# AIDynamicAction/rcognita

Hardware: AMD Instinct MI355X
Metric: env-control-steps/sec (whole node), 3wrobot Nactor=10 (higher is better)
Workload: dtype f64

## Files before the change

include/rcg.h:

```cpp
#ifndef RCG_H
#define RCG_H

#include <stdint.h>

#ifdef __cplusplus
extern "C" {
#endif

#define RCG_VERSION 124

#define RCG_MAX_DS 5
#define RCG_MAX_DU 2
#define RCG_MAX_CHI 7
#define RCG_MAX_PARS 5
#define RCG_MAX_DC 35
#define RCG_MAX_ROW 64
#define RCG_MAX_NACTOR 4096

typedef enum rcg_status {
  RCG_OK = 0,
  RCG_ERR_BAD_ARG = -1,
  RCG_ERR_HIP = -2,
  RCG_ERR_NO_DEVICE = -3,
  RCG_ERR_UNSUPPORTED = -4,
// ... 178 lines not shown
  RCG_KID_ACTOR = 1,
  RCG_KID_ACTOR_DMA = 2,
  RCG_KID_TICKS = 3,
  RCG_KID_ACTOR_OPT = 4,
  RCG_KID_NOMINAL = 5,
  RCG_KID_SIM = 6,
  RCG_KID_SIM_V = 7,
  RCG_KID_SIM_DIST = 8,
  RCG_KID_CRITIC_FIT = 9,
  RCG_KID_ACTOR_DMA_PACKED = 10,
  RCG_KID_ACTOR_SEARCH = 11,
  RCG_KID_COUNT_ = 12
} rcg_kernel_id;
int rcg_last_launch(const rcg_handle* h, int32_t kind, int32_t* kernel_id, int32_t* variant, int32_t* envs_per_wave);
int rcg_last_launch_zero_w(const rcg_handle* h, int32_t kind, uint32_t* mask);
const char* rcg_kernel_name(int32_t kernel_id);

#ifdef __cplusplus
}
#endif
#endif
```

rcognita_amd/_native.py:

```python
from __future__ import annotations

import ctypes as C
import os
import sys

_HERE = os.path.dirname(os.path.abspath(__file__))
LIB_PATH = os.path.join(_HERE, "lib", "librcg.so")

RCG_VERSION = 124
OK, ERR_BAD_ARG, ERR_HIP, ERR_NO_DEVICE, ERR_UNSUPPORTED, ERR_NONFINITE = 0, -1, -2, -3, -4, -5
SYS_3WROBOT, SYS_3WROBOT_NI, SYS_2TANK = 0, 1, 2
MODE_MPC, MODE_RQL, MODE_SQL = 0, 1, 2
STAGE_QUADRATIC, STAGE_BIQUADRATIC = 0, 1
CRITIC_QUAD_LIN, CRITIC_QUADRATIC, CRITIC_QUAD_NOMIX, CRITIC_QUAD_MIX = 0, 1, 2, 3
F32, F64 = 0, 1
HOST, DEVICE = 0, 1
FLAG_HAS_TARGET, FLAG_PER_ENV_PARS, FLAG_REF_LAG, FLAG_ACCUM_EVERY_SUBSTEP, FLAG_NO_CLIP = 1, 2, 4, 8, 16
FLAG_DISTURB = 32
DIM_DISTURB = {0: 2, 1: 2, 2: 1}

(FIELD_STATE, FIELD_ACTION, FIELD_ACCUM, FIELD_STEP_IDX, FIELD_EPISODE_IDX, FIELD_STATUS, FIELD_PARS,
 FIELD_STATE_INIT, FIELD_STATE_PREV, FIELD_BEST_J, FIELD_BEST_IDX, FIELD_W_CRITIC, FIELD_W_PREV, FIELD_OBS_BUF,
 FIELD_ACT_BUF, FIELD_RETURNS, FIELD_ACTION_SQN, FIELD_DISTURB, FIELD_SUBSTEP_IDX) = range(19)
FIELD_COUNT = 19
# ... 6 lines not shown
SYS_DIMS = {SYS_3WROBOT: (5, 2, 2), SYS_3WROBOT_NI: (3, 2, 0), SYS_2TANK: (2, 1, 5)}
SYS_DY = {}
SYS_USER_BASE = 16
MAX_DS, MAX_DU, MAX_PARS = 5, 2, 5

SYMBOLS = [
    "rcg_version", "rcg_last_error", "rcg_device_count", "rcg_create", "rcg_destroy", "rcg_set_stream", "rcg_use_own_stream",
    "rcg_synchronize", "rcg_dev_alloc", "rcg_dev_free", "rcg_memcpy_h2d", "rcg_memcpy_d2h", "rcg_set_field",
    "rcg_get_field", "rcg_field_bytes", "rcg_field_ptr", "rcg_rhs", "rcg_stage_obj", "rcg_critic",
    "rcg_actor_cost", "rcg_critic_cost", "rcg_sim_step", "rcg_sim_step_h", "rcg_actor_argmin", "rcg_control_tick",
    "rcg_critic_update", "rcg_control_ticks", "rcg_control_tick_n", "rcg_actor_optimize", "rcg_control_tick_opt", "rcg_nominal_action",
    "rcg_control_tick_nominal", "rcg_rhs_full", "rcg_disturb_noise", "rcg_episode_reset", "rcg_episode_stats", "rcg_tick_count", "rcg_set_tick_count", "rcg_profile", "rcg_profile_read",
    "rcg_profile_samples", "rcg_last_launch", "rcg_kernel_name", "rcg_wait_stream", "rcg_nominal_theta", "rcg_set_optimizer", "rcg_set_optimizer_tol", "rcg_set_tick_parts", "rcg_join", "rcg_loop_step", "rcg_loop_step_begin", "rcg_loop_step_end",
    "rcg_actor_search", "rcg_control_tick_search", "rcg_candidates_sample", "rcg_release_stream",
    "rcg_register_system", "rcg_rtc_version", "rcg_system_info", "rcg_system_output_info", "rcg_out",
    "rcg_system_has_critic", "rcg_system_programs", "rcg_critic_fit", "rcg_last_launch_zero_w", "rcg_system_has_search",
]
KERNEL_ACTOR, KERNEL_SIM, KERNEL_CRITIC = 0, 1, 2
(KID_NONE, KID_ACTOR, KID_ACTOR_DMA, KID_TICKS, KID_ACTOR_OPT, KID_NOMINAL, KID_SIM, KID_SIM_V, KID_SIM_DIST,
 KID_CRITIC_FIT, KID_ACTOR_DMA_PACKED, KID_ACTOR_SEARCH) = range(12)
DMA_MPC_G1, DMA_MPC, DMA_RQL_0, DMA_SQL_0 = 0, 1, 2, 6
LOOP_DECIDE, LOOP_PUSH, LOOP_FIT = 1, 2, 4
DMA_RQL_GEN_0 = 12
DMA_MPC_GEND, DMA_MPC_GENF = 10, 11


class RcgCfg(C.Structure):

    _fields_ = [
        ("struct_size", C.c_int32), ("sys_id", C.c_int32), ("batch", C.c_int32), ("dtype", C.c_int32),
        ("device", C.c_int32), ("n_actor", C.c_int32), ("mode", C.c_int32), ("stage_obj_struct", C.c_int32),
# ... 86 lines not shown
        "rcg_candidates_sample": (C.c_int, [vp, vp, i32, i32, vp]),
        "rcg_nominal_action": (C.c_int, [vp, vp, vp, vp, i32, C.c_double, C.POINTER(C.c_double), i32]),
        "rcg_control_tick_nominal": (C.c_int, [vp, C.c_double, C.POINTER(C.c_double)]),
        "rcg_nominal_theta": (C.c_int, [vp, vp, vp, i32]),
        "rcg_rhs_full": (C.c_int, [vp, vp, vp, vp, vp, vp, vp, vp, i32, i32]),
        "rcg_disturb_noise": (C.c_int, [vp, vp, vp]),
        "rcg_episode_reset": (C.c_int, [vp]),
        "rcg_episode_stats": (C.c_int, [vp, i32, vp, C.POINTER(RcgSummary)]),
        "rcg_tick_count": (i64, [vp]),
        "rcg_set_tick_count": (C.c_int, [vp, i64]),
        "rcg_profile": (C.c_int, [vp, i32]),
        "rcg_profile_read": (C.c_int, [vp, i32, C.POINTER(C.c_double), C.POINTER(i64)]),
        "rcg_profile_samples": (C.c_int, [vp, i32, C.POINTER(C.c_double), i64, C.POINTER(i64)]),
        "rcg_last_launch": (C.c_int, [vp, i32, C.POINTER(i32), C.POINTER(i32), C.POINTER(i32)]),
        "rcg_last_launch_zero_w": (C.c_int, [vp, i32, C.POINTER(C.c_uint32)]),
        "rcg_kernel_name": (C.c_char_p, [i32]),
        "rcg_wait_stream": (C.c_int, [vp, vp]),
        "rcg_release_stream": (C.c_int, [vp, vp]),
        "rcg_register_system": (C.c_int, [C.c_char_p, C.c_char_p, i32, i32, i32, C.POINTER(i32)]),
        "rcg_rtc_version": (C.c_int, [C.POINTER(i32), C.POINTER(i32)]),
        "rcg_system_info": (C.c_int, [i32, C.POINTER(i32), C.POINTER(i32), C.POINTER(i32), C.POINTER(i32)]),
        "rcg_system_output_info": (C.c_int, [i32, C.POINTER(i32), C.POINTER(i32), C.POINTER(i32)]),
        "rcg_out": (C.c_int, [vp, vp, vp, i32]),
        "rcg_system_has_critic": (C.c_int, [i32, C.POINTER(i32)]),
        "rcg_system_has_search": (C.c_int, [i32, C.POINTER(i32)]),
        "rcg_critic_fit": (C.c_int, [vp]),
        "rcg_system_programs": (C.c_int, [i32, C.c_char_p, i64, C.POINTER(i64)]),
    }
    for name, (res, args) in sig.items():
        fn = getattr(L, name)
# ... 55 lines not shown
```

rcognita_amd/csrc/rcg_actor_dma.hpp:

```cpp
#pragma once
#include <hip/hip_ext.h>
#include "rcg_kernels.hpp"

#ifndef RCG_DMA_AUX
#define RCG_DMA_AUX 2
#endif
#ifndef RCG_DMA_PRIO
#define RCG_DMA_PRIO 0
#endif

namespace rcg {

enum : int {
  DMA_MPC_G1 = 0,
  DMA_MPC = 1,
  DMA_RQL_0 = 2 ,
  DMA_SQL_0 = 6 ,
  DMA_MPC_GEND = 10,
  DMA_MPC_GENF = 11,
  DMA_RQL_GEN_0 = 12 ,
  DMA_VARIANTS = 16
};
__host__ __device__ constexpr bool dma_is_sql(int v) { return v >= DMA_SQL_0 && v < DMA_MPC_GEND; }
__host__ __device__ constexpr bool dma_is_rql(int v) { return (v >= DMA_RQL_0 && v < DMA_SQL_0) || v >= DMA_RQL_GEN_0; }
// ... 34 lines not shown
#else
  const double Jmin = wave_min_f64(bestJ);
  bestI = (int)wave_min_u32(bestJ == Jmin ? (unsigned)bestI : 0x7fffffffu);
  bestJ = Jmin;
#endif
}

template <typename Sys, typename real>
__host__ __device__ constexpr unsigned dma_zw_preset() {
  if constexpr (sizeof(real) == 8 && !HasOut<Sys>::value)
    return Sys::ZW_PRESET;
  else
    return 0u;
}

template <typename S, typename = void>
struct HasPrefix {
  static constexpr bool value = false;
};
template <typename S>
struct HasPrefix<S, void_t_<decltype(S::PFX_FREE)>> {
  static constexpr bool value = true;
};
template <typename S>
constexpr unsigned pfx_free() {
  if constexpr (HasPrefix<S>::value)
    return S::PFX_FREE;
  else
    return 0u;
}
template <typename S>
constexpr int pfx_heading() {
  if constexpr (HasPrefix<S>::value)
    return S::PFX_HEADING;
  else
    return -1;
}

__device__ __forceinline__ float uniform_r(float v) {
  return __uint_as_float((unsigned)__builtin_amdgcn_readfirstlane((int)__float_as_uint(v)));
}
__device__ __forceinline__ double uniform_r(double v) {
  const unsigned long long b = (unsigned long long)__double_as_longlong(v);
  const unsigned lo = (unsigned)__builtin_amdgcn_readfirstlane((int)(unsigned)b);
  const unsigned hi = (unsigned)__builtin_amdgcn_readfirstlane((int)(unsigned)(b >> 32));
  return __longlong_as_double((long long)(((unsigned long long)hi << 32) | lo));
}

template <int J, int NP, int SZ, int PIECE>
__device__ __forceinline__ void dma_pieces(const unsigned char* g, unsigned off, unsigned char* l) {
  typedef __attribute__((address_space(3))) void lds_void;
  typedef const __attribute__((address_space(1))) void glb_void;
  if constexpr (J < NP) {
    constexpr int BASE = (J * PIECE / 4096) * 4096;
    const unsigned char* const gb = g + (off + (unsigned)BASE);
    if constexpr (SZ == 16)
      __builtin_amdgcn_global_load_lds((glb_void*)gb, (lds_void*)(l + BASE), 16, J * PIECE - BASE, RCG_DMA_AUX);
    else
      __builtin_amdgcn_global_load_lds((glb_void*)gb, (lds_void*)(l + BASE), 4, J * PIECE - BASE, RCG_DMA_AUX);
    dma_pieces<J + 1, NP, SZ, PIECE>(g, off, l);
  }
}

__host__ __device__ constexpr int dma_rpl(int r, int esz) { return r * esz <= 24 ? 4 : (r * esz <= 32 ? 2 : 1); }

template <typename Sys, typename real, int R, bool TGT, int V, unsigned ZW = 0u>
__global__ __launch_bounds__(256) void k_actor_dma(const ActorArgs<real> A, const KParams<real> P) {
  constexpr int DS = Sys::DS, DY = sys_dy<Sys>(), DU = Sys::DU, NCHI = DY + DU, NP = Sys::NP;
  constexpr bool OUT = HasOut<Sys>::value;
  constexpr bool G1 = V == DMA_MPC_G1, SQL = dma_is_sql(V), RQL = dma_is_rql(V), CRIT = RQL || SQL;
  constexpr bool GEND = V == DMA_MPC_GEND, GENF = V == DMA_MPC_GENF, GEN = GEND || GENF;
  constexpr bool GENR = V >= DMA_RQL_GEN_0;
  static_assert(!(GEN || GENR) || TGT, "the generic-cost instances subtract a target (zeros for a handle without one)");
  static_assert(ZW == 0u || (G1 && sizeof(real) == 8 && !OUT && ZW == Sys::ZW_PRESET),
                "the zero-weight instance: DMA_MPC_G1, float64, no output map, the policy's preset mask");
  constexpr int CS = dma_cs(V);
  constexpr int DCMAX = CRIT ? dma_dc(CS, DY, DU) : 1;
  constexpr int ESZ = (int)sizeof(real);
  constexpr int WSLOT = dma_wslot(ESZ, V, DY, DU);
  constexpr bool WLDS = WSLOT > 0;
  constexpr int WREG = WLDS ? 1 : DCMAX;
  static_assert(R % DU == 0 && R >= DU && R <= 40, "row = N*du reals, at most 40 (f32: 160 bytes, f64: 320)");
  constexpr int N = R / DU;
  constexpr bool PFX = HasPrefix<Sys>::value && !OUT;
  constexpr unsigned FREE = PFX ? pfx_free<Sys>() : 0u;
  constexpr int HD = PFX ? pfx_heading<Sys>() : -1;
  constexpr bool TRIG0 = PFX && HD >= 0 && N >= 2;
  constexpr bool TRIG1 = TRIG0 && ((FREE >> (HD >= 0 ? HD : 0)) & 1u) && N >= 3;
  constexpr int RPL = dma_rpl(R, ESZ), TROWS = 64 * RPL;
  constexpr int TILE = TROWS * R * ESZ;
// ... 51 lines not shown
          __builtin_amdgcn_global_load_lds((glb_void*)(g + (o4 + (unsigned)(NFULL * 1024 + j * 256))),
                                           (lds_void*)(tile + NFULL * 1024 + j * 256), 4, 0, RCG_DMA_AUX);
    }
  };
  const int last_rows = rem_rows ? rem_rows : TROWS;
  auto rows_of = [&](int tt) -> int { return tt == T - 1 ? last_rows : TROWS; };

  real y0[DY], yn[sys_dxy<Sys>()], x0[DS], xn[DS], pv[NP > 0 ? NP : 1], pn[NP > 0 ? NP : 1], wc[WREG], wn[WREG];
  real wnl = 0;
  const bool lag = A.state_sys != A.obs;
#pragma unroll
  for (int i = 0; i < NP; ++i) pn[i] = P.pars[i];
#pragma unroll
  for (int i = 0; i < WREG; ++i) wn[i] = wc[i] = 0;
  constexpr int dc_rt = CRIT ? DCMAX : 0;
  auto fetch_env = [&](long b) {
    if (RCG_DBG(A, 4)) {
#pragma unroll
      for (int c = 0; c < sys_dxy<Sys>(); ++c) yn[c] = (real)0.5;
#pragma unroll
      for (int c = 0; c < DS; ++c) xn[c] = (real)0.5;
      return;
    }
    if constexpr (OUT) {
      load_obs_raw<Sys, real>(A.obs, A.obs_x, B, b, yn);
    } else {
#pragma unroll
      for (int c = 0; c < DS; ++c) yn[c] = A.obs[(long)c * B + b];
    }
    if (lag) {
#pragma unroll
// ... 66 lines not shown
#pragma unroll
  for (int c = 0; c < DS; ++c) x1s[c] = 0;
#pragma unroll
  for (int c = 0; c < DY; ++c) Sini[c] = 0;
  real bestJ = inf_r<real>();
  int bestI = 0x7fffffff;
  real bu[DU];
#pragma unroll
  for (int c = 0; c < DU; ++c) bu[c] = 0;
  real resJ = 0, resAcc = 0, resU[DU];
  int resI = 0;
#pragma unroll
  for (int c = 0; c < DU; ++c) resU[c] = 0;

  auto adopt_regs = [&]() {
    if constexpr (OUT) {
#pragma unroll
      for (int c = 0; c < DS; ++c) x0[c] = lag ? xn[c] : yn[c];
#pragma unroll
      for (int i = 0; i < NP; ++i) pv[i] = pn[i];
      pre_env = Sys::template prepare<real>(pv);
      obs_of_raw<Sys, real>(pre_env, A.obs_x, yn, y0);
    } else {
#pragma unroll
      for (int c = 0; c < DS; ++c) {
        y0[c] = yn[c];
        x0[c] = lag ? xn[c] : yn[c];
      }
    }
    if (CRIT && WLDS) {
      if (lane < dc_rt) wl[lane] = wnl;
      asm volatile("s_waitcnt lgkmcnt(0)" ::: "memory");
      __builtin_amdgcn_wave_barrier();
    } else if (CRIT) {
#pragma unroll
      for (int i = 0; i < WREG; ++i) wc[i] = wn[i];
    }
  };
  auto adopt_rest = [&]() {
    if constexpr (PFX) {
#pragma unroll
      for (int c = 0; c < DS; ++c) x0[c] = uniform_r(x0[c]);
      if constexpr (TRIG0) {
        sincos_sel<real, true>(x0[HD], &trig0[0], &trig0[1]);
        if constexpr (FREE != 0) {
          real uz[DU], d[DS];
#pragma unroll
          for (int c = 0; c < DU; ++c) uz[c] = 0;
          Sys::template rhs_trig<real>(pre_env, x0, uz, trig0[0], trig0[1], d);
#pragma unroll
          for (int c = 0; c < DS; ++c)
            if ((FREE >> c) & 1u) x1s[c] = uniform_r(fma_r(h, d[c], x0[c]));
        }
        if constexpr (TRIG1) {
          sincos_sel<real, true>(x1s[HD], &trig1[0], &trig1[1]);
          trig1[0] = uniform_r(trig1[0]);
          trig1[1] = uniform_r(trig1[1]);
        }
        if constexpr (FREE == 0) {
          trig0[0] = uniform_r(trig0[0]);
          trig0[1] = uniform_r(trig0[1]);
        }
      }
      if constexpr (G1) {
#pragma unroll
        for (int c = 0; c < DY; ++c) {
          if ((ZW >> c) & 1u) continue;
          const real chi0 = TGT ? y0[c] - P.target[c] : y0[c];
          real a = fma_r(chi0, chi0, (real)0);
          if (N >= 2 && ((FREE >> c) & 1u)) {
            const real chi1 = TGT ? x1s[c] - P.target[c] : x1s[c];
            a = fma_r(chi1, chi1, a);
          }
          Sini[c] = uniform_r(a);
        }
      }
    }
    if constexpr (ZW != 0u) {
      real z = 0;
#pragma unroll
      for (int i = 0; i < DY; ++i)
        if ((ZW >> i) & 1u) z = fma_r(P.R1d[i], y0[i] * y0[i], z);
      zw0 = uniform_r(z);
    }
    bestJ = inf_r<real>();
    bestI = 0x7fffffff;
  };
  const bool adopt_early = OUT || T == 1;

  for (int g = 0; g < n_tiles; ++g) {
    if (t == 0) {
      if constexpr (!OUT) {
        if (env_pars) pre_env = Sys::template prepare<real>(pn);
      }
      if (adopt_early) adopt_regs();
    }
    if constexpr (RCG_DMA_PRIO > 0 && ESZ == 8) __builtin_amdgcn_s_setprio(RCG_DMA_PRIO);
    asm volatile("s_waitcnt vmcnt(0)" ::: "memory");
    real rows[RPL][R];
#pragma unroll
    for (int j = 0; j < RPL; ++j) {
      const real* const myrow = reinterpret_cast<const real*>(tile) + (j * 64 + lane) * R;
#pragma unroll
      for (int i = 0; i < R; ++i) rows[j][i] = myrow[i];
    }
    asm volatile("s_waitcnt lgkmcnt(0)" ::: "memory");
    __builtin_amdgcn_wave_barrier();
// ... 207 lines not shown
```

rcognita_amd/csrc/rcg_api.hip:

```cpp
#include <cstdarg>
#include <cstdio>
#include <cstdlib>
#include <cstring>

#include "rcg_disturb.hpp"
#include "rcg_handle.hpp"
#include "rcg_search.hpp"

using namespace rcg;

static thread_local std::string g_err = "";

int rcg_fail(rcg_handle* h, int code, const char* fmt, ...) {
  char buf[512];
  va_list ap;
  va_start(ap, fmt);
  vsnprintf(buf, sizeof buf, fmt, ap);
  va_end(ap);
  if (h)
    h->err = buf;
  else
    g_err = buf;
  return code;
}
// ... 224 lines not shown
  h->dc = dim_critic(cfg->critic_struct, h->dy, du);
  h->esz = cfg->dtype == RCG_F64 ? 8 : 4;
  h->stream = nullptr;
  h->own_stream = nullptr;
  h->bounce = nullptr;
  h->tick_parts = 0;
  h->split_stream[0] = h->split_stream[1] = nullptr;
  h->split_fork = h->split_join[0] = h->split_join[1] = nullptr;
  h->split_pending = false;
  h->sub_lo = h->sub_hi = 0;
  h->probe = 0;
  h->d_summary = nullptr;
  h->d_const = nullptr;
  h->fit_scratch = nullptr;
  h->fit_scratch_bytes = 0;
  h->loop_seq = 0;
  h->loop_io.on = false;
  h->loop_pending = false;
  h->loop_pin = nullptr;
  h->sqn_alt = nullptr;
  h->loop_pending_decided = false;
  h->prof_mask = 0;
  h->prof_stride = 1;
  memset(h->prof_seen, 0, sizeof h->prof_seen);
  h->tick_count = 0;
  h->opt_ftol = 0.0;
  h->opt_memory = -1;
  h->cur_a = h->cur_b = nullptr;
  h->scope_due = false;
  h->order_ev = nullptr;
// ... 113 lines not shown
  if (h->own_stream) (void)hipStreamDestroy(h->own_stream);
  for (int p = 0; p < 2; ++p) {
    if (h->split_stream[p]) {
      (void)hipStreamSynchronize(h->split_stream[p]);
      (void)hipStreamDestroy(h->split_stream[p]);
    }
    if (h->split_join[p]) (void)hipEventDestroy(h->split_join[p]);
  }
  if (h->split_fork) (void)hipEventDestroy(h->split_fork);
  if (h->bounce) (void)hipHostFree(h->bounce);
  if (h->loop_pin) (void)hipHostFree(h->loop_pin);
  if (h->sqn_alt) (void)hipFree(h->sqn_alt);
  if (h->d_summary) (void)hipFree(h->d_summary);
  if (h->d_const) (void)hipFree(h->d_const);
  if (h->fit_scratch) (void)hipFree(h->fit_scratch);
  for (auto& p : h->ev_pending) {
    (void)hipEventDestroy(p.a);
    (void)hipEventDestroy(p.b);
  }
  for (auto e : h->ev_free) (void)hipEventDestroy(e);
  if (h->order_ev) (void)hipEventDestroy(h->order_ev);
  if (h->release_ev) (void)hipEventDestroy(h->release_ev);
  delete h;
  return RCG_OK;
}

int rcg_set_stream(rcg_handle* h, void* hip_stream) {
  DeviceGuard dev_guard(h);
  if (!h) return RCG_ERR_BAD_ARG;
  if ((hipStream_t)hip_stream == h->stream) return RCG_OK;
// ... 836 lines not shown

int rcg_last_launch(const rcg_handle* h, int32_t kind, int32_t* kernel_id, int32_t* variant, int32_t* envs_per_wave) {
  if (!h || kind < 0 || kind >= RCG_KERNEL_COUNT_) return RCG_ERR_BAD_ARG;
  if (kernel_id) *kernel_id = h->last[kind].kernel_id;
  if (variant) *variant = h->last[kind].variant;
  if (envs_per_wave) *envs_per_wave = h->last[kind].envs_per_wave;
  return RCG_OK;
}

int rcg_last_launch_zero_w(const rcg_handle* h, int32_t kind, uint32_t* mask) {
  if (!h || !mask || kind < 0 || kind >= RCG_KERNEL_COUNT_) return RCG_ERR_BAD_ARG;
  *mask = h->last[kind].zero_w;
  return RCG_OK;
}

const char* rcg_kernel_name(int32_t kernel_id) {
  static const char* const names[RCG_KID_COUNT_] = {"none",        "k_actor",   "k_actor_dma", "k_ticks",    "k_actor_opt",
                                                    "k_nominal",   "k_sim",     "k_sim_v",     "k_sim_dist", "k_critic_fit",
                                                    "k_actor_dma_packed", "k_actor_search"};
  return (kernel_id >= 0 && kernel_id < RCG_KID_COUNT_) ? names[kernel_id] : "?";
}

}
```

rcognita_amd/csrc/rcg_dma_launch.hpp:

```cpp
#pragma once

#include "rcg_actor_dma.hpp"
#include "rcg_actor_dma_packed.hpp"

namespace rcg {

template <typename Sys, typename real, int GROUP, int R>
static bool launch_dma_r(int r, int variant, dim3 grid, dim3 block, size_t lds, hipStream_t s, const ActorArgs<real>& A,
                         const KParams<real>& P, hipEvent_t ev_a, hipEvent_t ev_b) {
  if constexpr (R > dma_max_row<real>()) {
    return false;
  } else {
    if (r != R) return launch_dma_r<Sys, real, GROUP, R + 1>(r, variant, grid, block, lds, s, A, P, ev_a, ev_b);
    if constexpr (R % Sys::DU != 0) {
      return false;
    } else {
#define RCG_DMA_LAUNCH(FN)                                                                                           \
  {                                                                                                                  \
    auto fn = FN;                                                                                                    \
    if (lds > 64 * 1024)      \
      (void)hipFuncSetAttribute(reinterpret_cast<const void*>(fn), hipFuncAttributeMaxDynamicSharedMemorySize,       \
                                (int)lds);                                                                           \
    if (ev_a)                                                                                                        \
      hipExtLaunchKernelGGL(fn, grid, block, (std::uint32_t)lds, s, ev_a, ev_b, 0, A, P);                            \
    else                                                                                                             \
      hipLaunchKernelGGL(fn, grid, block, lds, s, A, P);                                                             \
    return true;                                                                                                     \
  }
#define RCG_DMA_CASE(V) \
  case V:               \
    RCG_DMA_LAUNCH((k_actor_dma<Sys, real, R, ((V) >= DMA_MPC_GEND ? true : Sys::TGT), V>))
      if constexpr (GROUP == 0) {
        constexpr unsigned ZWP = dma_zw_preset<Sys, real>();
        if constexpr (ZWP != 0u) {
          if (dma_zero_w<real>(ZWP, variant, A, P) != 0u) RCG_DMA_LAUNCH((k_actor_dma<Sys, real, R, Sys::TGT, DMA_MPC_G1, ZWP>))
        }
        switch (variant) {
          RCG_DMA_CASE(DMA_MPC_G1)
          RCG_DMA_CASE(DMA_MPC)
        }
      } else if constexpr (GROUP == 6) {
        switch (variant) {
          RCG_DMA_CASE(DMA_MPC_GEND)
          RCG_DMA_CASE(DMA_MPC_GENF)
        }
      } else if constexpr (GROUP == 7) {
        switch (variant) {
          RCG_DMA_CASE(DMA_RQL_GEN_0 + RCG_CRITIC_QUAD_LIN)
          RCG_DMA_CASE(DMA_RQL_GEN_0 + RCG_CRITIC_QUADRATIC)
          RCG_DMA_CASE(DMA_RQL_GEN_0 + RCG_CRITIC_QUAD_NOMIX)
// ... 92 lines not shown
```

rcognita_amd/csrc/rcg_handle.hpp:

```cpp
#pragma once
#include <hip/hip_ext.h>
#include <hip/hip_runtime.h>

#include <cstdint>
#include <cstdio>
#include <cstdlib>
#include <map>
#include <string>
#include <vector>

#include "rcg_actor_opt.hpp"
#include "rcg_kernels.hpp"

struct rcg_handle {
  rcg_cfg cfg;
  int ds, du, np, dc, nchi;
  int dy;
  bool rtc_has_out;
  size_t esz;
  hipStream_t stream;
  hipStream_t own_stream;
  void* f[RCG_FIELD_COUNT_];
  size_t fbytes[RCG_FIELD_COUNT_];
  double* d_summary;
// ... 3 lines not shown
  void* d_const;
  struct {
    bool on;
    const double* act_in;
    int n_substeps, dc;
    double *out, *flag, seq;
  } loop_io;
  bool loop_pending;
  int loop_pending_row;
  bool loop_pending_decided;
  void* sqn_alt;
  void* loop_pin;
  uint64_t loop_seq;
  void* fit_scratch;
  size_t fit_scratch_bytes;
  rcg::KParams<float> p32;
  rcg::KParams<double> p64;
  const struct SysVTable* sys;
  const struct RtcSystem* rtc;
  std::map<std::string, hipFunction_t> rtc_fn;
  std::string err;
  unsigned prof_mask;
  unsigned prof_stride;
  uint64_t prof_seen[RCG_KERNEL_COUNT_];
  std::vector<hipEvent_t> ev_free;
  struct Pending {
    hipEvent_t a, b;
    int kernel;
  };
  std::vector<Pending> ev_pending;
// ... 2 lines not shown
  std::vector<float> prof_samples[RCG_KERNEL_COUNT_];
  hipEvent_t cur_a, cur_b;
  bool scope_due;
  hipEvent_t order_ev;
  hipEvent_t release_ev;
  void* bounce;
  int tick_parts;
  hipStream_t split_stream[2];
  hipEvent_t split_fork, split_join[2];
  bool split_pending;
  int sub_lo, sub_hi;
  int probe;
  struct LastLaunch {
    int32_t kernel_id, variant, envs_per_wave;
    uint32_t zero_w;
  } last[RCG_KERNEL_COUNT_];
};
static constexpr size_t kProfMaxSamples = 65536;

static constexpr size_t kBounceBytes = 16384;
static constexpr int kSplitMinBatch = 65536;
static constexpr int kVariantSplitBit = 4096;
static inline void note_launch(rcg_handle* h, int kind, int kernel_id, int variant, int envs_per_wave) {
  h->last[kind].kernel_id = kernel_id;
  h->last[kind].variant = variant | (h->sub_hi > 0 ? kVariantSplitBit : 0);
  h->last[kind].envs_per_wave = envs_per_wave;
  h->last[kind].zero_w = 0u;
}

static constexpr size_t kConstR64 = 512, kConstW = 1296, kConstBytes = 2256;
static constexpr int kFitMaxRows = 8;

int rcg_fail(rcg_handle* h, int code, const char* fmt, ...);

#define HIPCHK(h, call)                                                                                 \
  do {                                                                                                  \
    hipError_t e_ = (call);                                                                             \
    if (e_ != hipSuccess)                                                                               \
      return rcg_fail((h), RCG_ERR_HIP, "%s failed: %s (%s:%d)", #call, hipGetErrorString(e_), __FILE__, \
                      __LINE__);                                                                        \
  } while (0)

// ... 142 lines not shown
```

rcognita_amd/csrc/rcg_kernels.hpp:

```cpp
#pragma once
#include <stdint.h>

#include <type_traits>

#include "../../include/rcg.h"
#include "rcg_systems.hpp"

namespace rcg {

enum : int { STAGE_FULL = 1, STAGE_BIQUAD = 2 };

#ifdef RCG_DEV
#define RCG_DBG(A, bit) ((A).dbg & (bit))
#else
#define RCG_DBG(A, bit) 0
#endif

template <typename real>
struct KParams {
  real pars[RCG_MAX_PARS];
  real lo[RCG_MAX_DU], hi[RCG_MAX_DU];
  const real* __restrict__ Rfull;
  real R1d[RCG_MAX_CHI], R2d[RCG_MAX_CHI];
  real target[RCG_MAX_DS];
// ... 272 lines not shown
  int G;
  int n_tiles;
  int grid_g;
  int vec_ok;
  int gpw;
  int jwave;
  int no_multi;
  int dbg;
  int env_lo, env_hi;
  real* sim_state;
  real* sim_state_prev;
  const real* sim_action;
  uint32_t* sim_status;
  int sim_n_sub;
  int obs_x;
};

typedef float v4f __attribute__((ext_vector_type(4)));

template <typename real>
__device__ __forceinline__ void stage_tile(const real* __restrict__ g, real* __restrict__ l, int n,
                                           int lane, int vec_ok) {
  if (vec_ok) {
    const int nv = (int)(((long)n * (long)sizeof(real)) >> 4);
    const v4f* __restrict__ gv = reinterpret_cast<const v4f*>(g);
    v4f* __restrict__ lv = reinterpret_cast<v4f*>(l);
    const int nfull = nv >> 6;
    for (int base = 0; base < nfull; base += 8) {
      const int cnt = nfull - base;
      v4f r[8];
// ... 693 lines not shown
  for (int c = 0; c < DU; ++c) u[c] = A.action[(long)c * B + b];
  const auto pre = load_pre<Sys, real>(P, A.pars_env, b);
  real accum = P.accum_every_substep ? A.accum[b] : (real)0;
  if (!env_substeps<Sys, real, TGT>(P, pre, A.n_sub, x, xp, u, st, accum)) {
    A.status[b] = st;
    return;
  }
#pragma unroll
  for (int c = 0; c < DS; ++c) {
    A.state[(long)c * B + b] = x[c];
    A.state_prev[(long)c * B + b] = xp[c];
  }
  if (P.accum_every_substep) A.accum[b] = accum;
}

template <typename Sys, typename real, bool TGT>
__global__ __launch_bounds__(256) void k_sim_v(const SimArgs<real> A, const KParams<real> P) {
  constexpr int DS = Sys::DS, DU = Sys::DU, NP = Sys::NP, VEC = 16 / (int)sizeof(real);
  typedef real vreal __attribute__((ext_vector_type(VEC)));
  typedef uint32_t vu32 __attribute__((ext_vector_type(VEC)));
  const long B = P.B;
  const long b0 = ((long)blockIdx.x * blockDim.x + threadIdx.x) * VEC;
  if (b0 >= B) return;
  vreal xv[DS], uv[DU], pv[NP > 0 ? NP : 1], av;
#pragma unroll
  for (int c = 0; c < DS; ++c) xv[c] = *reinterpret_cast<const vreal*>(A.state + (long)c * B + b0);
#pragma unroll
  for (int c = 0; c < DU; ++c) uv[c] = *reinterpret_cast<const vreal*>(A.action + (long)c * B + b0);
  const vu32 stv = *reinterpret_cast<const vu32*>(A.status + b0);
  if (A.pars_env) {
// ... 229 lines not shown
```

rcognita_amd/csrc/rcg_sysops.hpp:

```cpp
#pragma once
#include <cmath>
#include <cstdlib>
#include <cstring>
#include <type_traits>

#include "rcg_actor_dma.hpp"
#include "rcg_actor_dma_packed.hpp"
#include "rcg_critic_fit_ml.hpp"
#include "rcg_actor_opt.hpp"
#include "rcg_critic_fit.hpp"
#include "rcg_critic_fit_gen.hpp"
#include "rcg_disturb.hpp"
#include "rcg_handle.hpp"
#include "rcg_loop.hpp"
#include "rcg_nominal.hpp"
#include "rcg_search.hpp"
#include "rcg_ticks.hpp"

namespace rcg {

template <typename F>
static int by_dtype(rcg_handle* h, F&& f) {
  return h->cfg.dtype == RCG_F64 ? f(double{}) : f(float{});
}
// ... 543 lines not shown
  const bool generic = L.generic, tgt = L.tgt, dma_ok = L.dma_ok, pack_ok = L.pack_ok, fuse_sim = L.fuse_sim;
  if (h->probe == 1) {
    h->probe = (dma_ok && !pack_ok) ? 3 : 2;
    return RCG_OK;
  }
  if (h->sub_hi > 0 && !(dma_ok && !pack_ok))
    return rcg_fail(h, RCG_ERR_UNSUPPORTED, "%s: a split tick needs the k_actor_dma shape", who);
  if constexpr (std::is_same<real, float>::value && GenPk<Sys>::supported && GenPk<Sys>::fuse_tick) {
    if (tick && sim_first && !cand && !generic && !tgt && c.gamma == 1.0 && Sys::ZW_PRESET != 0u &&
        (P.zero_w & Sys::ZW_PRESET) == Sys::ZW_PRESET && K >= 256 && A.n_tiles % 4 == 0 && A.grid_g > 0 &&
        (64 % A.grid_g) == 0 && !A.no_multi && !knobs.no_pk && !knobs.no_tick_fuse && !(c.flags & RCG_FLAG_DISTURB) && !obs &&
        !state_sys &&
        action == h->f[RCG_FIELD_ACTION] && best_J == h->f[RCG_FIELD_BEST_J] && (void*)best_idx == h->f[RCG_FIELD_BEST_IDX])
      return op_ticks<Sys>(h, 1, K, nullptr);
  }
  if (sim_first && !fuse_sim) {
    int rc = op_sim_step<Sys>(h, c.substeps_per_tick);
    if (rc) return rc;
  }
  ProfScope prof_scope(h, RCG_KERNEL_ACTOR);
  if (pack_ok) {
    const ProfPair pp = prof_take(h);
    const ActorArgs<real> Ap = packed_args(h, A, L);
    const dim3 grid = L.pack_grid, block(256);
    const size_t lds_req = L.pack_lds;
    const bool launched =
        variant < DMA_RQL_0    ? launch_dma_packed<Sys, real, 3>(R, variant, grid, block, lds_req, h->stream, Ap, P, pp.a, pp.b)
        : variant >= DMA_SQL_0 ? launch_dma_packed<Sys, real, 4>(R, variant, grid, block, lds_req, h->stream, Ap, P, pp.a, pp.b)
                               : launch_dma_packed<Sys, real, 5>(R, variant, grid, block, lds_req, h->stream, Ap, P, pp.a, pp.b);
    if (launched) {
      note_launch(h, RCG_KERNEL_ACTOR, RCG_KID_ACTOR_DMA_PACKED, variant | (fuse_sim ? 16 : 0), (int)L.pack_gpw);
// ... 14 lines not shown
    const ProfPair pp = prof_take(h);
    if (variant >= DMA_RQL_GEN_0)
      ok = launch_dma<Sys, real, 7>(R, variant, grid, block, lds_req, h->stream, Ad, P, pp.a, pp.b);
    else if (variant >= DMA_MPC_GEND)
      ok = launch_dma<Sys, real, 6>(R, variant, grid, block, lds_req, h->stream, Ad, P, pp.a, pp.b);
    else if (variant < DMA_RQL_0)
      ok = launch_dma<Sys, real, 0>(R, variant, grid, block, lds_req, h->stream, Ad, P, pp.a, pp.b);
    else if (variant >= DMA_SQL_0)
      ok = launch_dma<Sys, real, 1>(R, variant, grid, block, lds_req, h->stream, Ad, P, pp.a, pp.b);
    else
      ok = launch_dma<Sys, real, 2>(R, variant, grid, block, lds_req, h->stream, Ad, P, pp.a, pp.b);
    if (!ok) prof_give_back(h, pp);
    if (ok) {
      note_launch(h, RCG_KERNEL_ACTOR, RCG_KID_ACTOR_DMA, variant, (int)L.dma_gpw);
      h->last[RCG_KERNEL_ACTOR].zero_w = dma_zero_w<real>(dma_zw_preset<Sys, real>(), variant, Ad, P);
      HIPCHK(h, hipGetLastError());
      return RCG_OK;
    }
  }
  if constexpr (std::is_same<real, float>::value && GenPk<Sys>::supported) {
    const bool pk_ok = !cand && !generic && !tgt && c.gamma == 1.0 && Sys::ZW_PRESET != 0u &&
                       (P.zero_w & Sys::ZW_PRESET) == Sys::ZW_PRESET && K >= 256 && A.n_tiles % 4 == 0 && A.grid_g > 0 &&
                       (64 % A.grid_g) == 0 && !A.no_multi && !knobs.no_pk;
    if (pk_ok) {
      RCG_LAUNCH(h, (k_actor<Sys, real, false, false, false, true>), dim3(blocks), dim3(64 * wpb), lds, A, P);
      note_launch(h, RCG_KERNEL_ACTOR, RCG_KID_ACTOR, 8, A.G);
      HIPCHK(h, hipGetLastError());
      return RCG_OK;
    }
  }
// ... 512 lines not shown
```

Measured before the change: 159.3 million.

## Precompute per-env actor prefix in the sim kernel as a packed env packet

Adds a k_sim_pkt kernel that, after stepping the simulation, computes the per-environment actor prefix (initial state, first predicted step, sin/cos of heading, initial stage-cost partials, zero-weight term) and writes it as a 16-double packet per env. The f64 zero-weight DMA actor kernel gets a PKT instance that loads this packet with one coalesced lane read plus readlane broadcasts, replacing its own state fetch and redundant per-wave prefix arithmetic. The prefix code is factored into a shared env_prefix helper. The cost is an extra device buffer and more bytes written by the sim kernel, and the path only applies under a narrow set of tick conditions.

```diff
diff --git a/include/rcg.h b/include/rcg.h
--- a/include/rcg.h
+++ b/include/rcg.h
@@ -7,7 +7,7 @@
 extern "C" {
 #endif
 
-#define RCG_VERSION 124
+#define RCG_VERSION 125
 
 #define RCG_MAX_DS 5
 #define RCG_MAX_DU 2
@@ -216,6 +216,7 @@
 } rcg_kernel_id;
 int rcg_last_launch(const rcg_handle* h, int32_t kind, int32_t* kernel_id, int32_t* variant, int32_t* envs_per_wave);
 int rcg_last_launch_zero_w(const rcg_handle* h, int32_t kind, uint32_t* mask);
+int rcg_last_launch_env_packet(const rcg_handle* h, int32_t kind);
 const char* rcg_kernel_name(int32_t kernel_id);
 
 #ifdef __cplusplus
diff --git a/rcognita_amd/_native.py b/rcognita_amd/_native.py
--- a/rcognita_amd/_native.py
+++ b/rcognita_amd/_native.py
@@ -7,7 +7,7 @@
 _HERE = os.path.dirname(os.path.abspath(__file__))
 LIB_PATH = os.path.join(_HERE, "lib", "librcg.so")
 
-RCG_VERSION = 124
+RCG_VERSION = 125
 OK, ERR_BAD_ARG, ERR_HIP, ERR_NO_DEVICE, ERR_UNSUPPORTED, ERR_NONFINITE = 0, -1, -2, -3, -4, -5
 SYS_3WROBOT, SYS_3WROBOT_NI, SYS_2TANK = 0, 1, 2
 MODE_MPC, MODE_RQL, MODE_SQL = 0, 1, 2
@@ -44,7 +44,7 @@
     "rcg_profile_samples", "rcg_last_launch", "rcg_kernel_name", "rcg_wait_stream", "rcg_nominal_theta", "rcg_set_optimizer", "rcg_set_optimizer_tol", "rcg_set_tick_parts", "rcg_join", "rcg_loop_step", "rcg_loop_step_begin", "rcg_loop_step_end",
     "rcg_actor_search", "rcg_control_tick_search", "rcg_candidates_sample", "rcg_release_stream",
     "rcg_register_system", "rcg_rtc_version", "rcg_system_info", "rcg_system_output_info", "rcg_out",
-    "rcg_system_has_critic", "rcg_system_programs", "rcg_critic_fit", "rcg_last_launch_zero_w", "rcg_system_has_search",
+    "rcg_system_has_critic", "rcg_system_programs", "rcg_critic_fit", "rcg_last_launch_zero_w", "rcg_last_launch_env_packet", "rcg_system_has_search",
 ]
 KERNEL_ACTOR, KERNEL_SIM, KERNEL_CRITIC = 0, 1, 2
 (KID_NONE, KID_ACTOR, KID_ACTOR_DMA, KID_TICKS, KID_ACTOR_OPT, KID_NOMINAL, KID_SIM, KID_SIM_V, KID_SIM_DIST,
@@ -161,6 +161,7 @@
         "rcg_profile_samples": (C.c_int, [vp, i32, C.POINTER(C.c_double), i64, C.POINTER(i64)]),
         "rcg_last_launch": (C.c_int, [vp, i32, C.POINTER(i32), C.POINTER(i32), C.POINTER(i32)]),
         "rcg_last_launch_zero_w": (C.c_int, [vp, i32, C.POINTER(C.c_uint32)]),
+        "rcg_last_launch_env_packet": (C.c_int, [vp, i32]),
         "rcg_kernel_name": (C.c_char_p, [i32]),
         "rcg_wait_stream": (C.c_int, [vp, vp]),
         "rcg_release_stream": (C.c_int, [vp, vp]),
diff --git a/rcognita_amd/csrc/rcg_actor_dma.hpp b/rcognita_amd/csrc/rcg_actor_dma.hpp
--- a/rcognita_amd/csrc/rcg_actor_dma.hpp
+++ b/rcognita_amd/csrc/rcg_actor_dma.hpp
@@ -72,28 +72,6 @@
     return 0u;
 }
 
-template <typename S, typename = void>
-struct HasPrefix {
-  static constexpr bool value = false;
-};
-template <typename S>
-struct HasPrefix<S, void_t_<decltype(S::PFX_FREE)>> {
-  static constexpr bool value = true;
-};
-template <typename S>
-constexpr unsigned pfx_free() {
-  if constexpr (HasPrefix<S>::value)
-    return S::PFX_FREE;
-  else
-    return 0u;
-}
-template <typename S>
-constexpr int pfx_heading() {
-  if constexpr (HasPrefix<S>::value)
-    return S::PFX_HEADING;
-  else
-    return -1;
-}
 
 __device__ __forceinline__ float uniform_r(float v) {
   return __uint_as_float((unsigned)__builtin_amdgcn_readfirstlane((int)__float_as_uint(v)));
@@ -122,7 +100,7 @@
 
 __host__ __device__ constexpr int dma_rpl(int r, int esz) { return r * esz <= 24 ? 4 : (r * esz <= 32 ? 2 : 1); }
 
-template <typename Sys, typename real, int R, bool TGT, int V, unsigned ZW = 0u>
+template <typename Sys, typename real, int R, bool TGT, int V, unsigned ZW = 0u, bool PKT = false>
 __global__ __launch_bounds__(256) void k_actor_dma(const ActorArgs<real> A, const KParams<real> P) {
   constexpr int DS = Sys::DS, DY = sys_dy<Sys>(), DU = Sys::DU, NCHI = DY + DU, NP = Sys::NP;
   constexpr bool OUT = HasOut<Sys>::value;
@@ -132,6 +110,8 @@
   static_assert(!(GEN || GENR) || TGT, "the generic-cost instances subtract a target (zeros for a handle without one)");
   static_assert(ZW == 0u || (G1 && sizeof(real) == 8 && !OUT && ZW == Sys::ZW_PRESET),
                 "the zero-weight instance: DMA_MPC_G1, float64, no output map, the policy's preset mask");
+  static_assert(!PKT || (ZW != 0u && env_pkt_ok<Sys, real>()), "the env-packet instance: the zero-weight instance of a policy with the hook");
+  using EP = EnvPkt<Sys, ZW>;
   constexpr int CS = dma_cs(V);
   constexpr int DCMAX = CRIT ? dma_dc(CS, DY, DU) : 1;
   constexpr int ESZ = (int)sizeof(real);
@@ -213,7 +193,15 @@
 #pragma unroll
   for (int i = 0; i < WREG; ++i) wn[i] = wc[i] = 0;
   constexpr int dc_rt = CRIT ? DCMAX : 0;
+  real pkn = 0;
   auto fetch_env = [&](long b) {
+    if constexpr (PKT) {
+      if (RCG_DBG(A, 4))
+        pkn = (real)0.5;
+      else if (lane < EP::STRIDE)
+        pkn = A.env_pkt[b * EP::STRIDE + lane];
+      return;
+    }
     if (RCG_DBG(A, 4)) {
 #pragma unroll
       for (int c = 0; c < sys_dxy<Sys>(); ++c) yn[c] = (real)0.5;
@@ -310,7 +298,23 @@
   for (int c = 0; c < DU; ++c) resU[c] = 0;
 
   auto adopt_regs = [&]() {
-    if constexpr (OUT) {
+    if constexpr (PKT) {
+#pragma unroll
+      for (int c = 0; c < DS; ++c) {
+        y0[c] = x0[c] = readlane_r(pkn, EP::X0 + c);
+        if (TRIG0 && ((FREE >> c) & 1u)) x1s[c] = readlane_r(pkn, EP::x1(c));
+        if (G1 && !((ZW >> c) & 1u)) Sini[c] = readlane_r(pkn, EP::sini(c));
+      }
+      if constexpr (TRIG0 && FREE == 0) {
+        trig0[0] = readlane_r(pkn, EP::TRIG0);
+        trig0[1] = readlane_r(pkn, EP::TRIG0 + 1);
+      }
+      if constexpr (TRIG1) {
+        trig1[0] = readlane_r(pkn, EP::TRIG1);
+        trig1[1] = readlane_r(pkn, EP::TRIG1 + 1);
+      }
+      zw0 = readlane_r(pkn, EP::ZW0);
+    } else if constexpr (OUT) {
 #pragma unroll
       for (int c = 0; c < DS; ++c) x0[c] = lag ? xn[c] : yn[c];
 #pragma unroll
@@ -334,51 +338,9 @@
     }
   };
   auto adopt_rest = [&]() {
-    if constexpr (PFX) {
-#pragma unroll
-      for (int c = 0; c < DS; ++c) x0[c] = uniform_r(x0[c]);
-      if constexpr (TRIG0) {
-        sincos_sel<real, true>(x0[HD], &trig0[0], &trig0[1]);
-        if constexpr (FREE != 0) {
-          real uz[DU], d[DS];
-#pragma unroll
-          for (int c = 0; c < DU; ++c) uz[c] = 0;
-          Sys::template rhs_trig<real>(pre_env, x0, uz, trig0[0], trig0[1], d);
-#pragma unroll
-          for (int c = 0; c < DS; ++c)
-            if ((FREE >> c) & 1u) x1s[c] = uniform_r(fma_r(h, d[c], x0[c]));
-        }
-        if constexpr (TRIG1) {
-          sincos_sel<real, true>(x1s[HD], &trig1[0], &trig1[1]);
-          trig1[0] = uniform_r(trig1[0]);
-          trig1[1] = uniform_r(trig1[1]);
-        }
-        if constexpr (FREE == 0) {
-          trig0[0] = uniform_r(trig0[0]);
-          trig0[1] = uniform_r(trig0[1]);
-        }
-      }
-      if constexpr (G1) {
-#pragma unroll
-        for (int c = 0; c < DY; ++c) {
-          if ((ZW >> c) & 1u) continue;
-          const real chi0 = TGT ? y0[c] - P.target[c] : y0[c];
-          real a = fma_r(chi0, chi0, (real)0);
-          if (N >= 2 && ((FREE >> c) & 1u)) {
-            const real chi1 = TGT ? x1s[c] - P.target[c] : x1s[c];
-            a = fma_r(chi1, chi1, a);
-          }
-          Sini[c] = uniform_r(a);
-        }
-      }
-    }
-    if constexpr (ZW != 0u) {
-      real z = 0;
-#pragma unroll
-      for (int i = 0; i < DY; ++i)
-        if ((ZW >> i) & 1u) z = fma_r(P.R1d[i], y0[i] * y0[i], z);
-      zw0 = uniform_r(z);
-    }
+    if constexpr (!PKT)
+      env_prefix<Sys, real, TGT, ZW, N, G1>(P, pre_env, h, x0, y0, x1s, trig0, trig1, Sini, zw0,
+                                            [](real v) { return uniform_r(v); });
     bestJ = inf_r<real>();
     bestI = 0x7fffffff;
   };
@@ -386,7 +348,7 @@
 
   for (int g = 0; g < n_tiles; ++g) {
     if (t == 0) {
-      if constexpr (!OUT) {
+      if constexpr (!OUT && !PKT) {
         if (env_pars) pre_env = Sys::template prepare<real>(pn);
       }
       if (adopt_early) adopt_regs();
diff --git a/rcognita_amd/csrc/rcg_api.hip b/rcognita_amd/csrc/rcg_api.hip
--- a/rcognita_amd/csrc/rcg_api.hip
+++ b/rcognita_amd/csrc/rcg_api.hip
@@ -262,6 +262,8 @@
   h->d_const = nullptr;
   h->fit_scratch = nullptr;
   h->fit_scratch_bytes = 0;
+  h->env_pkt = nullptr;
+  h->env_pkt_bytes = 0;
   h->loop_seq = 0;
   h->loop_io.on = false;
   h->loop_pending = false;
@@ -405,6 +407,7 @@
   if (h->d_summary) (void)hipFree(h->d_summary);
   if (h->d_const) (void)hipFree(h->d_const);
   if (h->fit_scratch) (void)hipFree(h->fit_scratch);
+  if (h->env_pkt) (void)hipFree(h->env_pkt);
   for (auto& p : h->ev_pending) {
     (void)hipEventDestroy(p.a);
     (void)hipEventDestroy(p.b);
@@ -1271,6 +1274,11 @@
   return RCG_OK;
 }
 
+int rcg_last_launch_env_packet(const rcg_handle* h, int32_t kind) {
+  if (!h || kind < 0 || kind >= RCG_KERNEL_COUNT_) return RCG_ERR_BAD_ARG;
+  return h->last[kind].env_pkt;
+}
+
 const char* rcg_kernel_name(int32_t kernel_id) {
   static const char* const names[RCG_KID_COUNT_] = {"none",        "k_actor",   "k_actor_dma", "k_ticks",    "k_actor_opt",
                                                     "k_nominal",   "k_sim",     "k_sim_v",     "k_sim_dist", "k_critic_fit",
diff --git a/rcognita_amd/csrc/rcg_dma_launch.hpp b/rcognita_amd/csrc/rcg_dma_launch.hpp
--- a/rcognita_amd/csrc/rcg_dma_launch.hpp
+++ b/rcognita_amd/csrc/rcg_dma_launch.hpp
@@ -33,7 +33,12 @@
       if constexpr (GROUP == 0) {
         constexpr unsigned ZWP = dma_zw_preset<Sys, real>();
         if constexpr (ZWP != 0u) {
-          if (dma_zero_w<real>(ZWP, variant, A, P) != 0u) RCG_DMA_LAUNCH((k_actor_dma<Sys, real, R, Sys::TGT, DMA_MPC_G1, ZWP>))
+          if (dma_zero_w<real>(ZWP, variant, A, P) != 0u) {
+            if constexpr (env_pkt_ok<Sys, real>()) {
+              if (A.env_pkt) RCG_DMA_LAUNCH((k_actor_dma<Sys, real, R, Sys::TGT, DMA_MPC_G1, ZWP, true>))
+            }
+            RCG_DMA_LAUNCH((k_actor_dma<Sys, real, R, Sys::TGT, DMA_MPC_G1, ZWP>))
+          }
         }
         switch (variant) {
           RCG_DMA_CASE(DMA_MPC_G1)
diff --git a/rcognita_amd/csrc/rcg_handle.hpp b/rcognita_amd/csrc/rcg_handle.hpp
--- a/rcognita_amd/csrc/rcg_handle.hpp
+++ b/rcognita_amd/csrc/rcg_handle.hpp
@@ -41,6 +41,8 @@
   uint64_t loop_seq;
   void* fit_scratch;
   size_t fit_scratch_bytes;
+  void* env_pkt;
+  size_t env_pkt_bytes;
   rcg::KParams<float> p32;
   rcg::KParams<double> p64;
   const struct SysVTable* sys;
@@ -73,6 +75,7 @@
   struct LastLaunch {
     int32_t kernel_id, variant, envs_per_wave;
     uint32_t zero_w;
+    int32_t env_pkt;
   } last[RCG_KERNEL_COUNT_];
 };
 static constexpr size_t kProfMaxSamples = 65536;
@@ -85,6 +88,7 @@
   h->last[kind].variant = variant | (h->sub_hi > 0 ? kVariantSplitBit : 0);
   h->last[kind].envs_per_wave = envs_per_wave;
   h->last[kind].zero_w = 0u;
+  h->last[kind].env_pkt = 0;
 }
 
 static constexpr size_t kConstR64 = 512, kConstW = 1296, kConstBytes = 2256;
diff --git a/rcognita_amd/csrc/rcg_kernels.hpp b/rcognita_amd/csrc/rcg_kernels.hpp
--- a/rcognita_amd/csrc/rcg_kernels.hpp
+++ b/rcognita_amd/csrc/rcg_kernels.hpp
@@ -310,6 +310,7 @@
   uint32_t* sim_status;
   int sim_n_sub;
   int obs_x;
+  const real* env_pkt;
 };
 
 typedef float v4f __attribute__((ext_vector_type(4)));
@@ -1033,6 +1034,161 @@
   if (P.accum_every_substep) A.accum[b] = accum;
 }
 
+template <typename S, typename = void>
+struct HasPrefix {
+  static constexpr bool value = false;
+};
+template <typename S>
+struct HasPrefix<S, void_t_<decltype(S::PFX_FREE)>> {
+  static constexpr bool value = true;
+};
+template <typename S>
+constexpr unsigned pfx_free() {
+  if constexpr (HasPrefix<S>::value)
+    return S::PFX_FREE;
+  else
+    return 0u;
+}
+template <typename S>
+constexpr int pfx_heading() {
+  if constexpr (HasPrefix<S>::value)
+    return S::PFX_HEADING;
+  else
+    return -1;
+}
+
+template <typename Sys, typename real, bool TGT, unsigned ZW, int N, bool G1, typename U>
+__device__ __forceinline__ void env_prefix(const KParams<real>& P, const typename Sys::template Pre<real>& pre_env, real h,
+                                           real* x0, const real* y0, real* x1s, real* trig0, real* trig1, real* Sini,
+                                           real& zw0, U uni) {
+  constexpr int DS = Sys::DS, DY = sys_dy<Sys>(), DU = Sys::DU;
+  constexpr bool PFX = HasPrefix<Sys>::value && !HasOut<Sys>::value;
+  constexpr unsigned FREE = PFX ? pfx_free<Sys>() : 0u;
+  constexpr int HD = PFX ? pfx_heading<Sys>() : -1;
+  constexpr bool TRIG0 = PFX && HD >= 0 && N >= 2;
+  constexpr bool TRIG1 = TRIG0 && ((FREE >> (HD >= 0 ? HD : 0)) & 1u) && N >= 3;
+  if constexpr (PFX) {
+#pragma unroll
+    for (int c = 0; c < DS; ++c) x0[c] = uni(x0[c]);
+    if constexpr (TRIG0) {
+      sincos_sel<real, true>(x0[HD], &trig0[0], &trig0[1]);
+      if constexpr (FREE != 0) {
+        real uz[DU], d[DS];
+#pragma unroll
+        for (int c = 0; c < DU; ++c) uz[c] = 0;
+        Sys::template rhs_trig<real>(pre_env, x0, uz, trig0[0], trig0[1], d);
+#pragma unroll
+        for (int c = 0; c < DS; ++c)
+          if ((FREE >> c) & 1u) x1s[c] = uni(fma_r(h, d[c], x0[c]));
+      }
+      if constexpr (TRIG1) {
+        sincos_sel<real, true>(x1s[HD], &trig1[0], &trig1[1]);
+        trig1[0] = uni(trig1[0]);
+        trig1[1] = uni(trig1[1]);
+      }
+      if constexpr (FREE == 0) {
+        trig0[0] = uni(trig0[0]);
+        trig0[1] = uni(trig0[1]);
+      }
+    }
+    if constexpr (G1) {
+#pragma unroll
+      for (int c = 0; c < DY; ++c) {
+        if ((ZW >> c) & 1u) continue;
+        const real chi0 = TGT ? y0[c] - P.target[c] : y0[c];
+        real a = fma_r(chi0, chi0, (real)0);
+        if (N >= 2 && ((FREE >> c) & 1u)) {
+          const real chi1 = TGT ? x1s[c] - P.target[c] : x1s[c];
+          a = fma_r(chi1, chi1, a);
+        }
+        Sini[c] = uni(a);
+      }
+    }
+  }
+  if constexpr (ZW != 0u) {
+    real z = 0;
+#pragma unroll
+    for (int i = 0; i < DY; ++i)
+      if ((ZW >> i) & 1u) z = fma_r(P.R1d[i], y0[i] * y0[i], z);
+    zw0 = uni(z);
+  }
+}
+
+template <typename Sys, unsigned ZW>
+struct EnvPkt {
+  static constexpr int popc(unsigned m, int n) {
+    int k = 0;
+    for (int i = 0; i < n; ++i) k += (int)((m >> i) & 1u);
+    return k;
+  }
+  static constexpr int DS = Sys::DS, STRIDE = 16;
+  static constexpr unsigned FREE = pfx_free<Sys>();
+  static constexpr int X0 = 0, X1 = DS, TRIG0 = X1 + popc(FREE, DS), TRIG1 = TRIG0 + 2, SINI = TRIG1 + 2,
+                       ZW0 = SINI + DS - popc(ZW, DS), LEN = ZW0 + 1;
+  static constexpr int x1(int c) { return X1 + popc(FREE, c); }
+  static constexpr int sini(int c) { return SINI + c - popc(ZW, c); }
+};
+template <typename Sys, typename real>
+__host__ __device__ constexpr bool env_pkt_ok() {
+  if constexpr (sizeof(real) == 8 && HasPrefix<Sys>::value && !HasOut<Sys>::value && Sys::DS > 2)
+    return Sys::ZW_PRESET != 0u && EnvPkt<Sys, Sys::ZW_PRESET>::LEN <= EnvPkt<Sys, Sys::ZW_PRESET>::STRIDE;
+  else
+    return false;
+}
+
+template <typename Sys, typename real, bool TGT, unsigned ZW, int NK>
+__global__ __launch_bounds__(256) void k_sim_pkt(const SimArgs<real> A, const KParams<real> P, real* __restrict__ pkt) {
+  constexpr int DS = Sys::DS, DU = Sys::DU;
+  using EP = EnvPkt<Sys, ZW>;
+  static_assert(sizeof(real) == 8 && EP::LEN <= EP::STRIDE && EP::STRIDE % 2 == 0, "float64 packets of 16 reals");
+  typedef real real2 __attribute__((ext_vector_type(2)));
+  const long b = (long)blockIdx.x * blockDim.x + threadIdx.x;
+  const long B = P.B;
+  if (b >= B) return;
+  uint32_t st = A.status[b];
+
+  real x[DS], xp[DS], u[DU];
+#pragma unroll
+  for (int c = 0; c < DS; ++c) xp[c] = x[c] = A.state[(long)c * B + b];
+#pragma unroll
+  for (int c = 0; c < DU; ++c) u[c] = A.action[(long)c * B + b];
+  const auto pre = load_pre<Sys, real>(P, A.pars_env, b);
+  if (!(st & 1u)) {
+    real accum = P.accum_every_substep ? A.accum[b] : (real)0;
+    if (!env_substeps<Sys, real, TGT>(P, pre, A.n_sub, x, xp, u, st, accum)) {
+      A.status[b] = st;
+    } else {
+#pragma unroll
+      for (int c = 0; c < DS; ++c) {
+        A.state[(long)c * B + b] = x[c];
+        A.state_prev[(long)c * B + b] = xp[c];
+      }
+      if (P.accum_every_substep) A.accum[b] = accum;
+    }
+  }
+  real pk[EP::STRIDE], x1s[DS], trig0[2] = {0, 0}, trig1[2] = {0, 0}, Sini[DS];
+  real zw0 = 0;
+#pragma unroll
+  for (int i = 0; i < EP::STRIDE; ++i) pk[i] = 0;
+#pragma unroll
+  for (int c = 0; c < DS; ++c) x1s[c] = Sini[c] = 0;
+  env_prefix<Sys, real, TGT, ZW, NK, true>(P, pre, P.h_pred, x, x, x1s, trig0, trig1, Sini, zw0, [](real v) { return v; });
+#pragma unroll
+  for (int c = 0; c < DS; ++c) {
+    pk[EP::X0 + c] = x[c];
+    if ((EP::FREE >> c) & 1u) pk[EP::x1(c)] = x1s[c];
+    if (!((ZW >> c) & 1u)) pk[EP::sini(c)] = Sini[c];
+  }
+  pk[EP::TRIG0] = trig0[0];
+  pk[EP::TRIG0 + 1] = trig0[1];
+  pk[EP::TRIG1] = trig1[0];
+  pk[EP::TRIG1 + 1] = trig1[1];
+  pk[EP::ZW0] = zw0;
+  real2* const dst = reinterpret_cast<real2*>(pkt + b * EP::STRIDE);
+#pragma unroll
+  for (int i = 0; i < EP::STRIDE / 2; ++i) dst[i] = real2{pk[2 * i], pk[2 * i + 1]};
+}
+
 template <typename Sys, typename real, bool TGT>
 __global__ __launch_bounds__(256) void k_sim_v(const SimArgs<real> A, const KParams<real> P) {
   constexpr int DS = Sys::DS, DU = Sys::DU, NP = Sys::NP, VEC = 16 / (int)sizeof(real);
diff --git a/rcognita_amd/csrc/rcg_sysops.hpp b/rcognita_amd/csrc/rcg_sysops.hpp
--- a/rcognita_amd/csrc/rcg_sysops.hpp
+++ b/rcognita_amd/csrc/rcg_sysops.hpp
@@ -581,7 +581,44 @@
         action == h->f[RCG_FIELD_ACTION] && best_J == h->f[RCG_FIELD_BEST_J] && (void*)best_idx == h->f[RCG_FIELD_BEST_IDX])
       return op_ticks<Sys>(h, 1, K, nullptr);
   }
-  if (sim_first && !fuse_sim) {
+  bool pkt = false;
+  if constexpr (env_pkt_ok<Sys, real>()) {
+#ifndef RCG_AB_NO_ENV_PACKET
+    pkt = tick && sim_first && !fuse_sim && !obs && !state_sys && !(c.flags & (RCG_FLAG_REF_LAG | RCG_FLAG_DISTURB)) &&
+          !h->f[RCG_FIELD_PARS] && dma_ok && !pack_ok && h->sub_hi == 0 && tgt == Sys::TGT &&
+          dma_zero_w<real>(dma_zw_preset<Sys, real>(), variant, A, P) != 0u;
+#endif
+    if (pkt) {
+      const size_t need = (size_t)c.batch * EnvPkt<Sys, Sys::ZW_PRESET>::STRIDE * sizeof(real);
+      if (h->env_pkt_bytes < need) {
+        if (h->env_pkt) (void)hipFree(h->env_pkt);
+        h->env_pkt = nullptr;
+        h->env_pkt_bytes = 0;
+        if (hipMalloc(&h->env_pkt, need) == hipSuccess)
+          h->env_pkt_bytes = need;
+        else
+          (void)hipGetLastError();
+      }
+      pkt = h->env_pkt != nullptr;
+    }
+    if (pkt) {
+      const SimArgs<real> S = sim_args<real>(h, c.substeps_per_tick);
+      constexpr unsigned ZWP = Sys::ZW_PRESET;
+      const dim3 grid(blocks_for(c.batch)), block(256);
+      ProfScope sim_scope(h, RCG_KERNEL_SIM);
+      if (c.n_actor >= 3)
+        RCG_LAUNCH(h, (k_sim_pkt<Sys, real, Sys::TGT, ZWP, 3>), grid, block, 0, S, P, (real*)h->env_pkt);
+      else if (c.n_actor == 2)
+        RCG_LAUNCH(h, (k_sim_pkt<Sys, real, Sys::TGT, ZWP, 2>), grid, block, 0, S, P, (real*)h->env_pkt);
+      else
+        RCG_LAUNCH(h, (k_sim_pkt<Sys, real, Sys::TGT, ZWP, 1>), grid, block, 0, S, P, (real*)h->env_pkt);
+      note_launch(h, RCG_KERNEL_SIM, RCG_KID_SIM, 0, 64);
+      h->last[RCG_KERNEL_SIM].env_pkt = 1;
+      HIPCHK(h, hipGetLastError());
+      A.env_pkt = (const real*)h->env_pkt;
+    }
+  }
+  if (sim_first && !fuse_sim && !pkt) {
     int rc = op_sim_step<Sys>(h, c.substeps_per_tick);
     if (rc) return rc;
   }
@@ -626,6 +663,7 @@
     if (ok) {
       note_launch(h, RCG_KERNEL_ACTOR, RCG_KID_ACTOR_DMA, variant, (int)L.dma_gpw);
       h->last[RCG_KERNEL_ACTOR].zero_w = dma_zero_w<real>(dma_zw_preset<Sys, real>(), variant, Ad, P);
+      h->last[RCG_KERNEL_ACTOR].env_pkt = Ad.env_pkt ? 1 : 0;
       HIPCHK(h, hipGetLastError());
       return RCG_OK;
     }
```

Result: slower. 157.5 million (-1.1%).
